# willake/cpu-ray-tracer

Measured on AMD Instinct MI355X. Metric: Mrays/sec (primary+secondary), 1280x720 64spp path trace — pipelined throughput over 878 consecutive 64-spp windows of one progressive render (single_render = one such render alone), higher is better.
Workload: dtype f32; 1 GPU; bunny_scene.xml FileScene BVH-SAH path tracer, 1280x720, 64 spp/step (passes=1, depthLimit=5); 1 step = 64 frames = the next spp window of a progressive render; the 878 steps are one crt_render job (14 render kernel launch(es), a wavefront per (tile, 128 consecutive frames), + ordered accumulate), one sync at the end; triangles=4968, parallelism=tile-wave x1

## Files before the change

cpu-ray-tracer_amd/csrc/device/render_pool.hip:

```cpp
#include <type_traits>
#include "launch.h"
#include "sample_body.h"

namespace crt {

enum : uint32_t {
    F_OX = 0, F_OY, F_OZ, F_DX, F_DY, F_DZ,
    F_RX, F_RY, F_RZ,
    F_T,
    F_SEED, F_META,
    F_U, F_V,
    F_COUNT,
    F_CUR = F_U, F_PEND = F_V,
    F_TRI = F_RX
};
constexpr uint32_t kMetaItemMask = 0x7ffu, kMetaDepthShift = 11u, kMetaInside = 1u << 14, kMetaFresh = 1u << 15, kMetaObjShift = 16u, kMetaLowMask = 0xffffu;
constexpr uint32_t kQueueMask = 127u;

#ifndef CRT_POOL_MIN_WAVES
#define CRT_POOL_MIN_WAVES 4
#endif
#ifndef CRT_POOL_WIDE_MIN_WAVES
#define CRT_POOL_WIDE_MIN_WAVES 4
#endif
#ifndef CRT_POOL_SHADE_MIN
#define CRT_POOL_SHADE_MIN 64
#endif
#ifndef CRT_POOL_NODE_STEPS
#define CRT_POOL_NODE_STEPS 2
#endif
#ifndef CRT_POOL_NODE2_MIN
#define CRT_POOL_NODE2_MIN 16
#endif
#ifndef CRT_POOL_STARVE
#define CRT_POOL_STARVE 40
#endif

#ifdef CRT_POOL_STAMPS
__device__ unsigned long long g_poolStamps[16];
#define CRT_PSTAMP(var) unsigned long long var; asm volatile("s_memtime %0\n\ts_waitcnt lgkmcnt(0)" : "=s"(var) :: "memory")
#define CRT_PACC(i, a, b) (pst[i] += (b) - (a))
#else
#define CRT_PSTAMP(var)
#define CRT_PACC(i, a, b)
#endif
#ifdef CRT_POOL_DENS
__device__ unsigned long long g_poolDens[48];
#define CRT_DENS(i, v) (dens[i] += (uint32_t)(v))
#define CRT_DENS_MASK(i, pred) (dens[i] += (uint32_t)__popcll(__builtin_amdgcn_ballot_w64(pred)))
#define CRT_LIVE_BUCKET(n) ((n) >= 112u ? 0u : (n) >= 96u ? 1u : (n) >= 64u ? 2u : 3u)
#else
#define CRT_DENS(i, v)
#define CRT_DENS_MASK(i, pred)
#endif
#ifdef CRT_POOL_TIMELINE
__device__ unsigned long long* g_poolTimeline = nullptr;
#endif
__device__ __forceinline__ bool lane_in(uint64_t m) { return __builtin_amdgcn_inverse_ballot_w64(m); }
__device__ __forceinline__ uint64_t finite3_mask(f3 v)
{
#ifdef CRT_DIET_NO_MASKS
    const uint32_t m = 0x7f800000u;
    return __builtin_amdgcn_ballot_w64((asu(v.x) & m) != m) & __builtin_amdgcn_ballot_w64((asu(v.y) & m) != m) & __builtin_amdgcn_ballot_w64((asu(v.z) & m) != m);
#else
    const float inf = __builtin_inff();
    return __builtin_amdgcn_fcmpf(__builtin_fabsf(v.x), inf, 4) & __builtin_amdgcn_fcmpf(__builtin_fabsf(v.y), inf, 4) & __builtin_amdgcn_fcmpf(__builtin_fabsf(v.z), inf, 4);
#endif
}
__device__ __forceinline__ uint32_t rank_in(uint64_t m) { return __builtin_amdgcn_mbcnt_hi((uint32_t)(m >> 32), __builtin_amdgcn_mbcnt_lo((uint32_t)m, 0u)); }

template <int KIND, bool COUNT, int S, int REFBITS = 16>
__global__ __launch_bounds__(64, REFBITS == 32 ? CRT_POOL_WIDE_MIN_WAVES : CRT_POOL_MIN_WAVES) void render_pool_kernel(const Scene sc, float4* __restrict__ slab, float* __restrict__ facScratch, Counters* __restrict__ counters,
                                                             unsigned long long* __restrict__ tileClocks, const uint32_t* __restrict__ tileOrder,
                                                             uint32_t tileFirst, uint32_t tileStride, uint32_t tileCount, uint32_t tilesX,
                                                             uint32_t sppFirst, uint32_t frames, uint32_t passes, uint32_t groups, uint32_t waveFrames, const uint32_t* __restrict__ waveTab, uint32_t tabBlocks, uint32_t longFrames,
                                                             uint32_t rankFirst, uint32_t* __restrict__ tileCost, unsigned long long* __restrict__ launchClk, const uint8_t* __restrict__ tileClass)
{
    extern __shared__ uint32_t lds[];
    const uint32_t lane = threadIdx.x;
#ifdef CRT_POOL_TIMELINE
    const unsigned long long tl0 = wall_clock64();
#endif
    const unsigned long long clk0 = (COUNT || tileCost) ? wall_clock64() : 0ull;
    if (launchClk && lane == 0) { atomicMax(&launchClk[0], ~clk0); atomicMax(&launchClk[1], clk0); }
    uint32_t rank0, grp, wf = waveFrames, first = 0u, limit = frames;
    if (waveTab) {
        if (blockIdx.x < tabBlocks) {
            uint32_t lo = 0u, hi = tileCount - rankFirst;
            while (hi - lo > 1u) { const uint32_t mid = (lo + hi) >> 1; if (waveTab[2u * mid] <= blockIdx.x) lo = mid; else hi = mid; }
            rank0 = lo; grp = blockIdx.x - waveTab[2u * lo]; wf = waveTab[2u * lo + 1u]; limit = longFrames;
        } else { const uint32_t b = blockIdx.x - tabBlocks; rank0 = b / groups; grp = b - rank0 * groups; wf = (uint32_t)S; first = longFrames; }
    } else { rank0 = blockIdx.x / groups; grp = blockIdx.x - rank0 * groups; }
    const uint32_t rank = rank0 + rankFirst;
    if (rank >= tileCount) return;
    const uint32_t tl = tileOrder ? tileOrder[rank] : rank;
    const uint32_t frame0 = first + grp * wf;
    if (frame0 >= limit) return;
    const uint32_t nOwn = (limit - frame0 < wf) ? limit - frame0 : wf;
    const uint32_t nStreams = nOwn < (uint32_t)S ? nOwn : (uint32_t)S;
    const uint32_t tile = tileFirst + tl * tileStride;
    const uint32_t tx = tile % tilesX, ty = tile / tilesX;
#ifdef CRT_NO_TILE_CLASS
    constexpr uint32_t tcls = 0u;
#else
    const uint32_t tcls = tileClass ? __builtin_amdgcn_readfirstlane((uint32_t)tileClass[tl]) : 0u;
#endif
    const bool skyTile = tcls == kTileSky;
    const char* __restrict__ geom = sc.geom;
    float* __restrict__ fac = facScratch + (size_t)blockIdx.x * (15u * (uint32_t)S);

    constexpr PoolRefForm R = pool_ref_form((uint32_t)REFBITS);
    using StackEntry = std::conditional_t<REFBITS == 32, uint32_t, uint16_t>;
    constexpr uint32_t kEntryB = (uint32_t)sizeof(StackEntry), kLevelB = 64u * kEntryB;
    char* const ldsB = reinterpret_cast<char*>(lds);
    const uint32_t laneB = lane * kEntryB;
    uint32_t* st = lds + (sc.stackDepth + 1u) * (kLevelB / 4u);
    float* stf = reinterpret_cast<float*>(st);
    uint8_t* qEnd = reinterpret_cast<uint8_t*>(st + F_COUNT * S);
    uint8_t* qBnc = qEnd + 128, * qRdy = qEnd + 256;
    uint16_t* slotFrame = reinterpret_cast<uint16_t*>(qEnd + 384);
    auto stk_top = [&](uint32_t at) -> uint32_t { return *reinterpret_cast<const StackEntry*>(ldsB + at); };
    auto stk_put = [&](uint32_t at, uint32_t v) { *reinterpret_cast<StackEntry*>(ldsB + at) = (StackEntry)v; };

    Cnt cn; cn.rays = cn.primary = cn.interior = cn.leaf = cn.tri = cn.tlas = cn.visits = cn.meshhits = 0;
    uint32_t trips = 0;
#ifdef CRT_POOL_DENS
    uint32_t dens[48]; for (int i = 0; i < 48; i++) dens[i] = 0;
    uint32_t live = nStreams; unsigned long long liveClk = wall_clock64();
#endif
    const uint32_t items = 256u * passes;
    const uint32_t rowLen = 64u * passes;
    const f3 nil3 = mk3(0.0f, 0.0f, 0.0f);

    for (uint32_t s = lane; s < nStreams; s += 64u) {
        st[F_SEED * S + s] = init_seed(tx + ty * (uint32_t)sc.W + (sppFirst + (frame0 + s) * passes) * 1799u);
        st[F_META * S + s] = kMetaFresh;
        qEnd[s] = (uint8_t)s;
        if (S > 64) slotFrame[s] = (uint16_t)s;
    }
    uint32_t nextFrame = nStreams;
    uint32_t endH = 0, endT = nStreams, bncH = 0, bncT = 0, rdyH = 0, rdyT = 0;

    uint64_t mRes = 0ull;
    uint64_t mFinite = ~0ull;
    uint32_t sid = 0, cur = kRefDone, spB = laneB, metaLo = 0u;
    f3 tO = nil3, tD = nil3, trD = nil3;
    Hit h; h.t = 1e34f; h.u = 0; h.v = 0; h.objIdx = -1; h.triIdx = -1;
    rec4 q0 = {0, 0, 0, 0}, q1 = q0, q2 = q0, q3 = q0;

    auto new_ray = [&](auto primary, bool act, uint32_t s, f3 v, bool norm, f3 O, uint32_t seed, uint32_t meta) {
#ifdef CRT_DIET_NO_CAMREL
        constexpr bool PRIM = false;
#else
        constexpr bool PRIM = decltype(primary)::value;
#endif
        constexpr bool FROM_CAM = decltype(primary)::value;
        const bool sky = FROM_CAM && skyTile;
        const bool noLight = FROM_CAM && (tcls & kTileNoLight) != 0u, noFloor = FROM_CAM && (tcls & kTileNoFloor) != 0u, noTree = FROM_CAM && (tcls & kTileNoTree) != 0u;
        f3 D = v, rD = v; Hit nh; nh.t = 1e34f; nh.u = 0; nh.v = 0; nh.objIdx = -1; nh.triIdx = -1;
        uint32_t ncur = kRefDone, pend = 0u;
        if (act) {
            const float inv = rcp_exact(sqrt_exact(dot3(v, v)));
            D = norm ? v * inv : v;
            cn.rays++;
            if (!sky) {
                rD = rcp_exact3(D);
                hit_light_floor<PRIM>(light_floor_from_kernarg<PRIM>(), O, D, nh, noLight, noFloor);
            }
            if (noTree) {
                if (COUNT) { if (KIND == 0) cn.interior++; else cn.tlas++; }
            } else if (sc.rootIsPair) {
                const kernarg_f rp = scene_floats(offsetof(Scene, rootPair));
                const rec4 a0 = {rp[0], rp[1], rp[2], rp[3]}, a1 = {rp[4], rp[5], rp[6], rp[7]};
                const rec4 b0 = {rp[8], rp[9], rp[10], rp[11]}, b1 = {rp[12], rp[13], rp[14], rp[15]};
                float d1, d2;
                const bool allFinite = (__builtin_amdgcn_ballot_w64(true) & ~finite3_mask(rD)) == 0ull;
                if constexpr (PRIM) {
                    const f3 ra0 = mk3(rp[16], rp[17], rp[18]), ra1 = mk3(rp[19], rp[20], rp[21]), rb0 = mk3(rp[22], rp[23], rp[24]), rb1 = mk3(rp[25], rp[26], rp[27]);
                    if (allFinite) { d1 = box_fast_rel(ra0, ra1, rD, nh.t); d2 = box_fast_rel(rb0, rb1, rD, nh.t); }
                    else { d1 = box_exact_rel(ra0, ra1, rD, nh.t); d2 = box_exact_rel(rb0, rb1, rD, nh.t); }
                } else if (allFinite) { d1 = box_fast(a0, a1, O, rD, nh.t); d2 = box_fast(b0, b1, O, rD, nh.t); }
                else { d1 = box_exact(a0, a1, O, rD, nh.t); d2 = box_exact(b0, b1, O, rD, nh.t); }
                const Ordered o = ordered_step(d1, d2, asu(a1.w), asu(b1.w));
                pend = o.push ? o.farRef : 0u;
                ncur = o.hitN ? o.nearRef : kRefDone;
                if (COUNT) { if (KIND == 0) cn.interior++; else cn.tlas++; }
            } else ncur = sc.rootRef16;
            if (COUNT && KIND == 0 && (ncur & R.tagMask) == 0u && ncur != kRefDone) cn.leaf++;
            if (!sky) {
                stf[F_OX * S + s] = O.x; stf[F_OY * S + s] = O.y; stf[F_OZ * S + s] = O.z;
                stf[F_RX * S + s] = rD.x; stf[F_RY * S + s] = rD.y; stf[F_RZ * S + s] = rD.z;
                stf[F_T * S + s] = nh.t;
                st[F_CUR * S + s] = ncur; st[F_PEND * S + s] = pend;
            }
            stf[F_DX * S + s] = D.x; stf[F_DY * S + s] = D.y; stf[F_DZ * S + s] = D.z;
            st[F_SEED * S + s] = seed; st[F_META * S + s] = meta | ((uint32_t)(nh.objIdx + 1) << kMetaObjShift);
        }
        const uint64_t mAct = __builtin_amdgcn_ballot_w64(act);
        uint64_t mW = 0ull, mE = mAct, mB = 0ull;
        if (!sky) {
            const uint32_t depth = (meta >> kMetaDepthShift) & 7u;
            mW = mAct & __builtin_amdgcn_ballot_w64(ncur != kRefDone);
            const uint64_t mStop = __builtin_amdgcn_ballot_w64((uint32_t)(nh.objIdx + 1) <= 1u) | __builtin_amdgcn_ballot_w64((int)depth >= sc.depthLimit);
            mE = mAct & ~mW & mStop; mB = mAct & ~mW & ~mStop;
        }
        CRT_DENS(20, __popcll(mAct)); CRT_DENS(19, __popcll(mW));
        if (!sky) {
            if (lane_in(mW)) qRdy[(rdyT + rank_in(mW)) & kQueueMask] = (uint8_t)s;
            if (lane_in(mB)) qBnc[(bncT + rank_in(mB)) & kQueueMask] = (uint8_t)s;
            rdyT += (uint32_t)__popcll(mW); bncT += (uint32_t)__popcll(mB);
        }
        if (lane_in(mE)) qEnd[(endT + rank_in(mE)) & kQueueMask] = (uint8_t)s;
        endT += (uint32_t)__popcll(mE);
    };
    auto world_ray = [&]() {
        tO = mk3(stf[F_OX * S + sid], stf[F_OY * S + sid], stf[F_OZ * S + sid]);
        tD = mk3(stf[F_DX * S + sid], stf[F_DY * S + sid], stf[F_DZ * S + sid]);
        trD = mk3(stf[F_RX * S + sid], stf[F_RY * S + sid], stf[F_RZ * S + sid]);
    };

    uint64_t mNode2 = 0ull;
    auto node_step = [&](uint64_t m) {
        const bool allFinite = (m & ~mFinite) == 0ull;
        if (lane_in(m)) {
            if (COUNT) { if (KIND == 1 && (cur & R.tlasBit) != 0u) cn.tlas++; else cn.interior++; }
            const uint32_t top = stk_top(spB);
            float d1, d2;
            if (__builtin_expect(allFinite, 1)) { d1 = box_fast(q0, q1, tO, trD, h.t); d2 = box_fast(q2, q3, tO, trD, h.t); }
            else { d1 = box_exact(q0, q1, tO, trD, h.t); d2 = box_exact(q2, q3, tO, trD, h.t); }
            const Ordered o = ordered_step(d1, d2, asu(q1.w), asu(q3.w));
            stk_put(spB + kLevelB, o.farRef);
            const bool pop = !o.hitN && spB != laneB;
            cur = o.hitN ? o.nearRef : (pop ? top : kRefDone);
            spB = spB + (o.push ? kLevelB : 0u) - (pop ? kLevelB : 0u);
            if (COUNT && (cur & R.tagMask) == 0u && cur != kRefDone) cn.leaf++;
        }
    };
    auto record_offset = [&]() -> uint32_t {
        const uint32_t idx = cur & R.indexMask;
        const bool inter = (cur & R.interior) != 0u;
        uint32_t oa = idx * (inter ? 64u : 48u) + (inter ? 0u : sc.leafOff - 48u);
        if (KIND == 1 && (cur & R.tlasBit) != 0u)
            oa = (cur & R.interior) ? sc.instOff + idx * 128u : sc.tlasPairOff + idx * 64u;
        return oa;
    };
    auto load_records = [&](uint64_t m) {
        const uint32_t oa = record_offset();
        if (lane_in(m)) { q0 = ldp<0>(geom, oa); q1 = ldp<1>(geom, oa); q2 = ldp<2>(geom, oa); q3 = ldp<3>(geom, oa); }
    };

    auto tri_step = [&](uint64_t m) {
        CRT_DENS(3, 1); CRT_DENS(4, __popcll(m));
        if (lane_in(m)) {
            if (COUNT) cn.tri++;
            const uint32_t top = stk_top(spB);
            hit_tri(q0, q1, q2, tO, tD, h);
            const bool more = asu(q2.w) > 1u;
            const bool pop = !more && spB != laneB;
            const uint32_t next = more ? cur + 1u : (pop ? top : kRefDone);
            spB -= pop ? kLevelB : 0u;
            if (COUNT && !more && (next & R.tagMask) == 0u && next != kRefDone) cn.leaf++;
            cur = next;
        }
    };

#ifdef CRT_POOL_STAMPS
    unsigned long long pst[12] = {0, 0, 0, 0, 0, 0, 0, 0, 0, 0, 0, 0};
#endif
    for (;;) {
        CRT_PSTAMP(p0);
        if (mRes != 0ull) {
            uint64_t mNode, mTlas = 0ull;
            if (KIND == 0) mNode = mRes & __builtin_amdgcn_ballot_w64(cur > R.interior - 1u);
            else { mTlas = mRes & __builtin_amdgcn_ballot_w64(cur >= R.tlasLeaf); mNode = mRes & __builtin_amdgcn_ballot_w64(cur - R.tlasBit < R.interior); }
            const uint64_t mTri = mRes & ~(mNode | mTlas);
            asm volatile("" : "+v"(q0), "+v"(q1), "+v"(q2), "+v"(q3));
            CRT_DENS(22, __popcll(mRes));
            if (mNode) { CRT_DENS(1, 1); CRT_DENS(2, __popcll(mNode)); }

            if (KIND == 1 && mTlas) { CRT_DENS(23, 1); CRT_DENS(24, __popcll(mTlas)); }
            uint64_t mBack = 0ull;
            if (KIND == 1 && mTlas != 0ull) {
                if (lane_in(mTlas)) {
                    if (COUNT) { cn.tlas++; cn.visits++; }
                    const f3 O = mk3(stf[F_OX * S + sid], stf[F_OY * S + sid], stf[F_OZ * S + sid]);
                    const f3 D = mk3(stf[F_DX * S + sid], stf[F_DY * S + sid], stf[F_DZ * S + sid]);
                    to_object_space(q0, q1, q2, O, D, tO, tD, trD);
                    spB += kLevelB; stk_put(spB, R.ret);
                    const uint32_t next = asu(q3.y);
                    if (COUNT && (next & R.tagMask) == 0u && next != kRefDone) cn.leaf++;
                    cur = next;
                }
                mFinite = (mFinite & ~mTlas) | (mTlas & finite3_mask(trD));
            }
            if (mNode != 0ull) node_step(mNode);
#if CRT_POOL_NODE_STEPS > 1
            uint64_t mLeafNow = 0ull;
#pragma unroll
            for (int rep = 1; rep < CRT_POOL_NODE_STEPS; rep++) {
                const uint64_t mStepped = rep == 1 ? mNode : mNode2;
                mNode2 = mStepped & (KIND == 0 ? __builtin_amdgcn_ballot_w64(cur > R.interior - 1u) : __builtin_amdgcn_ballot_w64(cur - R.tlasBit < R.interior));
                if ((uint32_t)__popcll(mNode2) < (uint32_t)CRT_POOL_NODE2_MIN) { mNode2 = 0ull; break; }
                const uint64_t mLeaf = mStepped & __builtin_amdgcn_ballot_w64((cur & R.tagMask) == 0u) & ~__builtin_amdgcn_ballot_w64(cur == kRefDone);
                load_records(mNode2 | mLeaf);
                mLeafNow |= mLeaf;
                CRT_DENS(28, 1); CRT_DENS(29, __popcll(mNode2));
                node_step(mNode2);
            }
            const uint64_t mTriAll = mTri | mLeafNow;
            const uint64_t mTriRan = mTriAll;
#else
            const uint64_t mTriAll = mTri;
            const uint64_t mTriRan = mTriAll;
#endif
            if (mTriAll != 0ull) tri_step(mTriAll);
            if (KIND == 1) {
                mBack = (mNode | mTriRan) & __builtin_amdgcn_ballot_w64(cur == R.ret);
                if (mBack != 0ull) {
                    if (lane_in(mBack)) {
                        world_ray();
                        const bool pop = spB != laneB;
                        const uint32_t top = stk_top(spB);
                        cur = pop ? top : kRefDone; spB -= pop ? kLevelB : 0u;
                        if (COUNT && (cur & R.tagMask) == 0u && cur != kRefDone) cn.leaf++;
                    }
                    mFinite = (mFinite & ~mBack) | (mBack & finite3_mask(trD));
                }
            }
            asm volatile("" ::: "memory");
            const uint64_t mFin = mRes & __builtin_amdgcn_ballot_w64(cur == kRefDone);
            if (mFin != 0ull) {
                CRT_DENS(5, 1); CRT_DENS(6, __popcll(mFin));
                const uint32_t depth = (metaLo >> kMetaDepthShift) & 7u;
                const uint64_t mStop = __builtin_amdgcn_ballot_w64((uint32_t)(h.objIdx + 1) <= 1u) | __builtin_amdgcn_ballot_w64((int)depth >= sc.depthLimit);
                const uint64_t mE = mFin & mStop, mB = mFin & ~mStop;
                if (lane_in(mFin)) {
                    stf[F_T * S + sid] = h.t; stf[F_U * S + sid] = h.u; stf[F_V * S + sid] = h.v;
                    st[F_TRI * S + sid] = (uint32_t)h.triIdx;
                    st[F_META * S + sid] = metaLo | ((uint32_t)(h.objIdx + 1) << kMetaObjShift);
                }
                if (lane_in(mE)) qEnd[(endT + rank_in(mE)) & kQueueMask] = (uint8_t)sid;
                if (lane_in(mB)) qBnc[(bncT + rank_in(mB)) & kQueueMask] = (uint8_t)sid;
                endT += (uint32_t)__popcll(mE); bncT += (uint32_t)__popcll(mB);
                mRes &= ~mFin;
            }
            asm volatile("" ::: "memory");
        }
        CRT_PSTAMP(p1); CRT_PACC(0, p0, p1);
        if (__builtin_expect(mRes == 0ull, 0)) {
            if ((endT - endH) + (bncT - bncH) + (rdyT - rdyH) == 0u) break;
        }
        if (COUNT) trips++;
        CRT_DENS(0, 1);
#ifdef CRT_POOL_DENS
        dens[32u + CRT_LIVE_BUCKET(live)]++;
#endif
        {
            const uint32_t nRdy = rdyT - rdyH;
            const uint64_t mFree = ~mRes;
            if (nRdy != 0u) if (mFree != 0ull) {
                const uint32_t myRank = rank_in(mFree);
                const uint64_t mTake = mFree & __builtin_amdgcn_ballot_w64(myRank < nRdy);
                CRT_DENS(7, 1); CRT_DENS(8, __popcll(mTake));
                if (lane_in(mTake)) {
                    sid = qRdy[(rdyH + myRank) & kQueueMask];
                    tO = mk3(stf[F_OX * S + sid], stf[F_OY * S + sid], stf[F_OZ * S + sid]);
                    tD = mk3(stf[F_DX * S + sid], stf[F_DY * S + sid], stf[F_DZ * S + sid]);
                    trD = mk3(stf[F_RX * S + sid], stf[F_RY * S + sid], stf[F_RZ * S + sid]);
                    const uint32_t meta = st[F_META * S + sid];
                    h.t = stf[F_T * S + sid]; h.objIdx = (int)(meta >> kMetaObjShift) - 1; h.u = 0; h.v = 0; h.triIdx = -1;
                    metaLo = meta & kMetaLowMask;
                    cur = st[F_CUR * S + sid];
                    const uint32_t pend = st[F_PEND * S + sid];
                    stk_put(laneB + kLevelB, pend);
                    spB = laneB + (pend ? kLevelB : 0u);
                }
                mFinite = (mFinite & ~mTake) | (mTake & finite3_mask(trD));
                mRes |= mTake;
                rdyH += (uint32_t)__popcll(mTake);
            }
            if (mRes != 0ull) {
                CRT_DENS(21, 1);
                uint32_t oa = record_offset();
                if (!lane_in(mRes)) oa = 0u;
                q0 = ldp<0>(geom, oa); q1 = ldp<1>(geom, oa); q2 = ldp<2>(geom, oa); q3 = ldp<3>(geom, oa);
            }
        }
        asm volatile("" ::: "memory");
        {
            const uint32_t nEnd = endT - endH, nBnc = bncT - bncH, nRdy = rdyT - rdyH, nRes = (uint32_t)__popcll(mRes);
            const bool starving = nRes + nRdy < (uint32_t)CRT_POOL_STARVE;
            bool runEnd = false, runBnc = false;
            if ((nEnd | nBnc) >= (uint32_t)CRT_POOL_SHADE_MIN || starving) {
                runEnd = nEnd >= (uint32_t)CRT_POOL_SHADE_MIN || (starving && nEnd > 0u && nEnd >= nBnc);
                runBnc = nBnc >= (uint32_t)CRT_POOL_SHADE_MIN || (starving && nBnc > nEnd);
            }

            CRT_PSTAMP(p2b); CRT_PACC(1, p1, p2b);
            if (runEnd) {
                const uint32_t n = nEnd < 64u ? nEnd : 64u;
                const bool act = lane < n;
                const uint32_t s = act ? qEnd[(endH + lane) & kQueueMask] : 0u;
                endH += n;
                uint32_t meta = 0, seed = 0; int obj = -1; f3 D = nil3;
                if (act) { meta = st[F_META * S + s]; seed = st[F_SEED * S + s]; obj = (int)(meta >> kMetaObjShift) - 1; D = mk3(stf[F_DX * S + s], stf[F_DY * S + s], stf[F_DZ * S + s]); }
                const bool first = (meta & kMetaFresh) != 0u;
                const int depth = (int)((meta >> kMetaDepthShift) & 7u);
                uint32_t item = meta & kMetaItemMask;
                const bool ended = act && !first, miss = ended && obj == -1;
#ifdef CRT_POOL_DENS
                dens[36u + CRT_LIVE_BUCKET(live)]++;
#endif
                CRT_DENS(9, 1); CRT_DENS(10, n); CRT_DENS_MASK(11, miss); CRT_DENS_MASK(13, act && first); CRT_DENS_MASK(25, ended && depth > 0); CRT_DENS_MASK(26, ended && depth > 1); CRT_DENS_MASK(27, ended && depth > 2);
                if (ended && obj >= 2) cn.meshhits++;
                float fk[15];
#pragma unroll
                for (int k = 0; k < 5; k++) {
                    fk[3 * k] = fk[3 * k + 1] = fk[3 * k + 2] = 0.0f;
                    if (!skyTile) if (ended && depth > k) {
#pragma unroll
                        for (int j = 0; j < 3; j++) fk[3 * k + j] = __hip_atomic_load(fac + (3 * k + j) * S + s, __ATOMIC_RELAXED, __HIP_MEMORY_SCOPE_AGENT);
                    }
                }
                uint32_t skyTexel = 0u;
                if (miss) {
                    float phi, theta; sky_angles(D, phi, theta);
                    const kernarg_f sk = scene_floats(offsetof(Scene, skyOffset));
                    skyTexel = sc.texels[tex_index(asu(sk[0]), (int)asu(sk[1]), (int)asu(sk[2]), phi * CRT_INV2PI, theta * CRT_INVPI)];
                }
                bool gen = act && first;
                size_t sampleAt = 0;
                if (ended) {
                    uint32_t pix = item, pass = 0;
                    if (passes != 1u) { pix = item / passes; pass = item - pix * passes; }
                    const uint32_t fr = frame0 + (S > 64 ? (uint32_t)slotFrame[s] : s);
                    sampleAt = (((size_t)(fr >> 6) * tileCount + tl) * 256u + pix) * rowLen + ((fr & 63u) * passes + pass);
                    item++;
                    gen = item < items;
                }
                if (S > 64) if (nextFrame < nOwn) {
                    const uint64_t mDone = __builtin_amdgcn_ballot_w64(ended) & ~__builtin_amdgcn_ballot_w64(gen);
                    if (mDone != 0ull) {
                        const uint32_t f = nextFrame + rank_in(mDone);
                        const uint64_t mTake = mDone & __builtin_amdgcn_ballot_w64(f < nOwn);
                        if (lane_in(mTake)) {
                            slotFrame[s] = (uint16_t)f;
                            seed = init_seed(tx + ty * (uint32_t)sc.W + (sppFirst + (frame0 + f) * passes) * 1799u);
                            item = 0u; gen = true;
                        }
                        nextFrame += (uint32_t)__popcll(mTake);
                    }
                }
#ifdef CRT_POOL_DENS
                {
                    const uint32_t gone = (uint32_t)__popcll(__builtin_amdgcn_ballot_w64(ended) & ~__builtin_amdgcn_ballot_w64(gen));
                    if (gone) { const unsigned long long now = wall_clock64(); dens[44u + CRT_LIVE_BUCKET(live)] += (uint32_t)(now - liveClk); liveClk = now; live -= gone; }
                }
#endif
                const kernarg_f cam = scene_floats(offsetof(Scene, camPos));
                const f3 camPos = mk3(cam[0], cam[1], cam[2]);
                f3 v = camPos;
                if (gen) {
                    const uint32_t pix = (passes == 1u) ? item : item / passes;
                    const f3 TL = mk3(cam[3], cam[4], cam[5]);
#ifdef CRT_DIET_NO_CAMREL
                    const f3 TR = mk3(cam[6], cam[7], cam[8]), BL = mk3(cam[9], cam[10], cam[11]);
                    const f3 right = TR - TL, down = BL - TL;
#else
                    constexpr size_t pc = (offsetof(Scene, primRight) - offsetof(Scene, camPos)) / 4;
                    const f3 right = mk3(cam[pc], cam[pc + 1], cam[pc + 2]), down = mk3(cam[pc + 3], cam[pc + 4], cam[pc + 5]);
#endif
                    v = primary_target(camPos, TL, right, down, cam[12], cam[13], tx, ty, pix, seed);
                    cn.primary++;
                }
                CRT_DENS_MASK(12, gen);
                CRT_PSTAMP(e1); CRT_PACC(2, p2b, e1);
                new_ray(std::true_type{}, gen, s, v, true, camPos, seed, item);
                CRT_PSTAMP(e2); CRT_PACC(3, e1, e2);
                if (ended) {
                    f3 L = miss ? tex_unpack(skyTexel) : ((depth >= sc.depthLimit) ? mk3(0, 0, 0) : mk3(24, 24, 22));
                    if (!skyTile) {
#pragma unroll
                        for (int k = 4; k >= 0; k--)
                            if (depth > k) L = mk3(fk[3 * k], fk[3 * k + 1], fk[3 * k + 2]) * L;
                    }
                    slab[sampleAt] = make_float4(L.x, L.y, L.z, 0.0f);
                }
#ifdef CRT_POOL_STAMPS
                { CRT_PSTAMP(e3); CRT_PACC(4, e2, e3); pst[10]++; }
#endif
                asm volatile("" :: "v"(fk[0]), "v"(fk[1]), "v"(fk[2]), "v"(fk[3]), "v"(fk[4]), "v"(fk[5]), "v"(fk[6]), "v"(fk[7]), "v"(fk[8]), "v"(fk[9]), "v"(fk[10]), "v"(fk[11]), "v"(fk[12]), "v"(fk[13]), "v"(fk[14]), "v"(skyTexel));
            }
            CRT_PSTAMP(p3);
            asm volatile("" ::: "memory");
            if (runBnc) {
                const uint32_t n = nBnc < 64u ? nBnc : 64u;
                const bool act = lane < n;
                const uint32_t s = act ? qBnc[(bncH + lane) & kQueueMask] : 0u;
                bncH += n;
                f3 O = nil3, D = nil3; float ht = 0, hu = 0, hv = 0; int obj = 1; uint32_t tri = 0, seed = 0, meta = 0;
                if (act) {
                    tri = st[F_TRI * S + s];
                    O = mk3(stf[F_OX * S + s], stf[F_OY * S + s], stf[F_OZ * S + s]);
                    D = mk3(stf[F_DX * S + s], stf[F_DY * S + s], stf[F_DZ * S + s]);
                    ht = stf[F_T * S + s]; hu = stf[F_U * S + s]; hv = stf[F_V * S + s];
                    seed = st[F_SEED * S + s]; meta = st[F_META * S + s]; obj = (int)(meta >> kMetaObjShift) - 1;
                }
                const bool mesh = act && obj >= 2;
#ifdef CRT_POOL_DENS
                dens[40u + CRT_LIVE_BUCKET(live)]++;
#endif
                CRT_DENS(14, 1); CRT_DENS(15, n); CRT_DENS_MASK(16, mesh);
                rec4 s0 = {0, 0, 0, 0}, s1 = s0, s2 = s0, s3 = s0;
                if (mesh) { const uint32_t so = sc.shadeOff + tri * 64u; s0 = ldp<0>(geom, so); s1 = ldp<1>(geom, so); s2 = ldp<2>(geom, so); s3 = ldp<3>(geom, so); cn.meshhits++; }
                const bool inside = (meta & kMetaInside) != 0u;
                const int depth = (int)((meta >> kMetaDepthShift) & 7u);
                const uint32_t item = meta & kMetaItemMask;
                f3 v = O; bool newInside = false;
                if (act) {
                    const f3 I = O + ht * D;
                    SurfPoint p;
                    if (obj == 1) {
                        const kernarg_f fl = scene_floats(offsetof(Scene, floorN));
                        const kernarg_f fm = scene_floats(offsetof(Scene, floorMat));
                        const rec4 m0 = {fm[0], fm[1], fm[2], fm[3]}, m1 = {fm[4], fm[5], fm[6], fm[7]};
                        p = floor_point(mk3(fl[0], fl[1], fl[2]), fl[4], m0, m1, I);
                    } else p = mesh_point<KIND>(s0, s1, s2, s3, hu, hv, obj, geom, sc.instOff, sc.mats);
                    const f3 N = face_ray(p.N, D);
                    uint32_t texel = 0x00ffffffu;
                    if (p.tW > 0) texel = sc.texels[tex_index(p.tOff, p.tW, p.tH, p.tu, p.tv)];
                    const f3 medium = medium_of(inside, p.absorb, ht);
                    CRT_PSTAMP(b1); CRT_PACC(5, p3, b1);
                    const Bounce b = draw_bounce(seed, D, N, inside, p.refl, p.refr);
                    newInside = b.newInside;
                    const f3 c = (p.tW > 0) ? tex_unpack(texel) : mk3(1.0f, 1.0f, 1.0f);
                    CRT_PSTAMP(b2); CRT_PACC(6, b1, b2);
                    const float inv = rcp_exact(sqrt_exact(dot3(b.v, b.v)));
                    const f3 nv = b.branch == kDiffuse ? b.v * inv : b.v;
                    v = nv;
                    const f3 factor = bounce_factor(b.branch, c, medium, nv, N);
                    float* fd = fac + (3 * depth) * S + s;
                    __hip_atomic_store(fd, factor.x, __ATOMIC_RELAXED, __HIP_MEMORY_SCOPE_AGENT);
                    __hip_atomic_store(fd + S, factor.y, __ATOMIC_RELAXED, __HIP_MEMORY_SCOPE_AGENT);
                    __hip_atomic_store(fd + 2 * S, factor.z, __ATOMIC_RELAXED, __HIP_MEMORY_SCOPE_AGENT);
                    O = I + nv * CRT_EPS;
                    CRT_PSTAMP(b3); CRT_PACC(7, b2, b3);
                }
                CRT_PSTAMP(b4);
                new_ray(std::false_type{}, act, s, v, false, O, seed, item | ((uint32_t)(depth + 1) << kMetaDepthShift) | (newInside ? kMetaInside : 0u));
#ifdef CRT_POOL_STAMPS
                { CRT_PSTAMP(b5); CRT_PACC(8, b4, b5); pst[11]++; }
#endif
                asm volatile("" :: "v"(s0), "v"(s1), "v"(s2), "v"(s3));
            }
#ifdef CRT_POOL_STAMPS
            pst[9]++;
#endif
        }
    }
#ifdef CRT_POOL_STAMPS
    if (lane == 0) for (int i = 0; i < 12; i++) atomicAdd(&g_poolStamps[i], pst[i]);
#endif
#ifdef CRT_POOL_DENS
    dens[44u + CRT_LIVE_BUCKET(live)] += (uint32_t)(wall_clock64() - liveClk);
    if (lane == 0) for (int i = 0; i < 48; i++) if (dens[i]) atomicAdd(&g_poolDens[i], (unsigned long long)dens[i]);
#endif

#ifdef CRT_POOL_TIMELINE
    if (lane == 0 && g_poolTimeline) { uint32_t hw; asm volatile("s_getreg_b32 %0, hwreg(HW_REG_HW_ID)" : "=s"(hw)); g_poolTimeline[3 * (size_t)blockIdx.x] = tl0; g_poolTimeline[3 * (size_t)blockIdx.x + 1] = wall_clock64(); g_poolTimeline[3 * (size_t)blockIdx.x + 2] = hw; }
#endif
    if (tileCost && lane == 0 && nOwn == (uint32_t)S) atomicMax(&tileCost[tl], (uint32_t)((wall_clock64() - clk0) * 64ull / (uint32_t)S));
    if (launchClk && lane == 0) { const unsigned long long now = wall_clock64(), last = __hip_atomic_load(&launchClk[1], __ATOMIC_RELAXED, __HIP_MEMORY_SCOPE_AGENT), from = last > clk0 ? last : clk0; if (now > from) atomicAdd(&launchClk[2], now - from); }
    if (COUNT && tileClocks && lane == 0 && nOwn == frames) {
        tileClocks[2 * tl] = wall_clock64() - clk0;
        tileClocks[2 * tl + 1] = trips;
    }
    uint32_t vals[8] = {cn.rays, cn.primary, cn.interior, cn.leaf, cn.tri, cn.tlas, cn.visits, cn.meshhits};
#pragma unroll
    for (int i = 0; i < 8; i++) {
        if (!COUNT && i >= 2 && i != 7) continue;
        uint32_t sum = wave_sum(vals[i]);
        if (lane == 0 && sum) atomicAdd(&counters->v[i], (unsigned long long)sum);
    }
}

}

#ifndef CRT_POOL_STREAMS
#define CRT_POOL_STREAMS 128
#endif
extern "C" uint32_t crt_pool_streams(uint32_t frames) { return frames > 64u ? (uint32_t)CRT_POOL_STREAMS : 64u; }
#ifndef CRT_POOL_EXTRA_LDS
#define CRT_POOL_EXTRA_LDS 0
#endif
extern "C" uint32_t crt_pool_lds_bytes(uint32_t stackDepth, uint32_t streams, uint32_t refBits) { return (stackDepth + 1u) * 64u * (refBits / 8u) + crt::F_COUNT * streams * 4u + 3u * 128u + (streams > 64u ? 2u * streams : 0u) + (uint32_t)CRT_POOL_EXTRA_LDS; }
extern "C" uint32_t crt_pool_lds_limit(int device)
{
    static uint32_t known[64] = {};
    if (device >= 0 && device < 64 && known[device]) return known[device];
    int v = 0;
    if (hipDeviceGetAttribute(&v, hipDeviceAttributeMaxSharedMemoryPerBlock, device) != hipSuccess || v <= 0) { (void)hipGetLastError(); return 0u; }
    const uint32_t limit = (uint32_t)v < 64u * 1024u ? (uint32_t)v : 64u * 1024u;
    if (device >= 0 && device < 64) known[device] = limit;
    return limit;
}
extern "C" size_t crt_pool_scratch_bytes_per_window(uint32_t tileCount) { return (size_t)tileCount * 128u * 15u * 4u; }

#ifdef CRT_POOL_STAMPS
extern "C" int crt_debug_pool_stamps(unsigned long long* out, int reset)
{
    if (out && hipMemcpyFromSymbol(out, HIP_SYMBOL(crt::g_poolStamps), 128) != hipSuccess) return -1;
    if (reset) { unsigned long long z[16] = {}; if (hipMemcpyToSymbol(HIP_SYMBOL(crt::g_poolStamps), z, 128) != hipSuccess) return -1; }
    return 0;
}
#endif
#ifdef CRT_POOL_DENS
extern "C" int crt_debug_pool_density(unsigned long long* out, int reset)
{
    if (out && hipMemcpyFromSymbol(out, HIP_SYMBOL(crt::g_poolDens), 384) != hipSuccess) return -1;
    if (reset) { unsigned long long z[48] = {}; if (hipMemcpyToSymbol(HIP_SYMBOL(crt::g_poolDens), z, 384) != hipSuccess) return -1; }
    return 0;
}
#endif
#ifdef CRT_POOL_TIMELINE
static unsigned long long* g_timelineHost = nullptr; static size_t g_timelineCount = 0;
extern "C" size_t crt_debug_pool_timeline(unsigned long long* out, size_t cap)
{
    const size_t n = g_timelineCount < cap ? g_timelineCount : cap;
    if (out && n) (void)hipMemcpy(out, g_timelineHost, n * 24, hipMemcpyDeviceToHost);
    return g_timelineCount;
}
#endif
extern "C" hipError_t crt_launch_render_pool(const crt::Scene* sc, void* slab, void* facScratch, crt::Counters* counters, unsigned long long* tileClocks, const uint32_t* tileOrder,
                                             uint32_t tileFirst, uint32_t tileStride, uint32_t tileCount, uint32_t tilesX, uint32_t sppFirst,
                                             uint32_t frames, uint32_t passes, int collectStats, uint32_t rankFirst, uint32_t waveFrames, const uint32_t* waveTab, uint32_t tabBlocks, uint32_t longFrames,
                                             uint32_t* tileCost, unsigned long long* launchClk, const uint8_t* tileClass, uint32_t extraLds, hipStream_t stream)
{
    if (tileCount == 0 || frames == 0) return hipSuccess;
    if (sc->poolRefBits != 16u && sc->poolRefBits != 32u) return hipErrorInvalidValue;
    const uint32_t S = crt_pool_streams(frames);
    const uint32_t wf = (S == 64u || waveFrames < S) ? S : waveFrames;
    if (wf % S != 0u || wf > 0xff80u) return hipErrorInvalidValue;
    if (S == 64u) waveTab = nullptr;
    if (waveTab && (tabBlocks == 0u || longFrames == 0u || longFrames > frames)) return hipErrorInvalidValue;
    const uint32_t groups = waveTab ? (frames - longFrames + S - 1u) / S : (frames + wf - 1u) / wf;
    if ((unsigned long long)tileCount * ((frames + S - 1u) / S) > 0x7fffffffull) return hipErrorInvalidValue;
    if (rankFirst >= tileCount) return hipSuccess;
    dim3 grid(waveTab ? tabBlocks + (tileCount - rankFirst) * groups : (tileCount - rankFirst) * groups), block(64);
#ifdef CRT_POOL_TIMELINE
    { static unsigned long long* buf = nullptr; static size_t cap = 0;
      if (cap < (size_t)grid.x) { if (buf) (void)hipFree(buf); (void)hipMalloc((void**)&buf, (size_t)grid.x * 24); cap = grid.x; (void)hipMemcpyToSymbol(HIP_SYMBOL(crt::g_poolTimeline), &buf, sizeof(buf)); }
      (void)hipMemsetAsync(buf, 0, (size_t)grid.x * 24, stream); g_timelineHost = buf; g_timelineCount = grid.x; }
#endif
    const uint32_t ldsBytes = crt_pool_lds_bytes(sc->stackDepth, S, sc->poolRefBits) + extraLds;
    { int dev = 0; if (hipGetDevice(&dev) != hipSuccess) return hipGetLastError(); if (ldsBytes > crt_pool_lds_limit(dev)) return hipErrorInvalidValue; }
#define CRT_LAUNCH(K, C, SS) do { if (sc->poolRefBits == 32u) CRT_LAUNCH_R(K, C, SS, 32); else CRT_LAUNCH_R(K, C, SS, 16); } while (0)
#define CRT_LAUNCH_R(K, C, SS, RB) hipLaunchKernelGGL((crt::render_pool_kernel<K, C, SS, RB>), grid, block, ldsBytes, stream, *sc, (float4*)slab, (float*)facScratch, counters, tileClocks, tileOrder, tileFirst, tileStride, tileCount, tilesX, sppFirst, frames, passes, groups, wf, waveTab, tabBlocks, longFrames, rankFirst, tileCost, launchClk, tileClass)
#define CRT_LAUNCH_S(K, C) do { if (S == 64u) CRT_LAUNCH(K, C, 64); else CRT_LAUNCH(K, C, CRT_POOL_STREAMS); } while (0)
    if (sc->kind == 0) { if (collectStats) CRT_LAUNCH_S(0, true); else CRT_LAUNCH_S(0, false); }
    else { if (collectStats) CRT_LAUNCH_S(1, true); else CRT_LAUNCH_S(1, false); }
#undef CRT_LAUNCH_S
#undef CRT_LAUNCH
#undef CRT_LAUNCH_R
    return hipGetLastError();
}
```

Before: 31340 Mrays/s.

## Keep wavefront pool control decisions scalar and specialize node steps on finiteness

Reworks the persistent pool kernel's control flow so lane masks come straight from scalar compares (uicmp/sicmp) rather than ballots over per-lane bools. Sky checks, pass counts and the shading-pass decision are pinned into SGPRs. The node traversal is split into two compiled variants, one assuming all inverse directions are finite (the common case) and one exact fallback. A live-stream counter replaces the queue-empty exit check, and the end-pass refill logic is restructured around masks. The aim is to cut VALU and ballot overhead and divergent branching in the scheduler loop, at the cost of code duplication and some subtle correctness risk in the rewritten termination logic.

```diff
diff --git a/cpu-ray-tracer_amd/csrc/device/render_pool.hip b/cpu-ray-tracer_amd/csrc/device/render_pool.hip
--- a/cpu-ray-tracer_amd/csrc/device/render_pool.hip
+++ b/cpu-ray-tracer_amd/csrc/device/render_pool.hip
@@ -67,6 +67,19 @@
     return __builtin_amdgcn_fcmpf(__builtin_fabsf(v.x), inf, 4) & __builtin_amdgcn_fcmpf(__builtin_fabsf(v.y), inf, 4) & __builtin_amdgcn_fcmpf(__builtin_fabsf(v.z), inf, 4);
 #endif
 }
+#define CRT_CTL_SEQ() asm volatile("")
+__device__ __forceinline__ bool ctl_free(uint64_t mRes) { CRT_CTL_SEQ(); return mRes != ~0ull; }
+#ifdef CRT_CTL_NO_DECIDE
+__device__ __forceinline__ uint32_t fresh(uint32_t x) { return x; }
+#else
+__device__ __forceinline__ uint32_t fresh(uint32_t x) { asm("" : "+s"(x)); return x; }
+#endif
+__device__ __forceinline__ uint32_t pop32(uint64_t m) { uint32_t n = (uint32_t)__builtin_popcountll(m); asm("" : "+s"(n)); return n; }
+__device__ __forceinline__ uint64_t mask_ne(uint32_t a, uint32_t b) { return __builtin_amdgcn_uicmp(a, b, 33); }
+__device__ __forceinline__ uint64_t mask_eq(uint32_t a, uint32_t b) { return __builtin_amdgcn_uicmp(a, b, 32); }
+__device__ __forceinline__ uint64_t mask_ult(uint32_t a, uint32_t b) { return __builtin_amdgcn_uicmp(a, b, 36); }
+__device__ __forceinline__ uint64_t mask_ule(uint32_t a, uint32_t b) { return __builtin_amdgcn_uicmp(a, b, 37); }
+__device__ __forceinline__ uint64_t mask_sge(int a, int b) { return __builtin_amdgcn_sicmp(a, b, 39); }
 __device__ __forceinline__ uint32_t rank_in(uint64_t m) { return __builtin_amdgcn_mbcnt_hi((uint32_t)(m >> 32), __builtin_amdgcn_mbcnt_lo((uint32_t)m, 0u)); }
 
 template <int KIND, bool COUNT, int S, int REFBITS = 16>
@@ -105,7 +118,12 @@
 #else
     const uint32_t tcls = tileClass ? __builtin_amdgcn_readfirstlane((uint32_t)tileClass[tl]) : 0u;
 #endif
+#if defined(CRT_CTL_NO_DECIDE) || defined(CRT_NO_TILE_CLASS)
     const bool skyTile = tcls == kTileSky;
+    auto not_sky = [&]() -> bool { return !skyTile; };
+#else
+    auto not_sky = [&]() -> bool { return fresh(tcls) != kTileSky; };
+#endif
     const char* __restrict__ geom = sc.geom;
     float* __restrict__ fac = facScratch + (size_t)blockIdx.x * (15u * (uint32_t)S);
 
@@ -138,6 +156,9 @@
         qEnd[s] = (uint8_t)s;
         if (S > 64) slotFrame[s] = (uint16_t)s;
     }
+#ifndef CRT_CTL_NO_DECIDE
+    uint32_t nLive = nStreams;
+#endif
     uint32_t nextFrame = nStreams;
     uint32_t endH = 0, endT = nStreams, bncH = 0, bncT = 0, rdyH = 0, rdyT = 0;
 
@@ -148,14 +169,13 @@
     Hit h; h.t = 1e34f; h.u = 0; h.v = 0; h.objIdx = -1; h.triIdx = -1;
     rec4 q0 = {0, 0, 0, 0}, q1 = q0, q2 = q0, q3 = q0;
 
-    auto new_ray = [&](auto primary, bool act, uint32_t s, f3 v, bool norm, f3 O, uint32_t seed, uint32_t meta) {
+    auto new_ray = [&](auto primary, uint64_t mActIn, bool act, uint32_t s, f3 v, bool norm, f3 O, uint32_t seed, uint32_t meta) {
 #ifdef CRT_DIET_NO_CAMREL
         constexpr bool PRIM = false;
 #else
         constexpr bool PRIM = decltype(primary)::value;
 #endif
         constexpr bool FROM_CAM = decltype(primary)::value;
-        const bool sky = FROM_CAM && skyTile;
         const bool noLight = FROM_CAM && (tcls & kTileNoLight) != 0u, noFloor = FROM_CAM && (tcls & kTileNoFloor) != 0u, noTree = FROM_CAM && (tcls & kTileNoTree) != 0u;
         f3 D = v, rD = v; Hit nh; nh.t = 1e34f; nh.u = 0; nh.v = 0; nh.objIdx = -1; nh.triIdx = -1;
         uint32_t ncur = kRefDone, pend = 0u;
@@ -163,7 +183,7 @@
             const float inv = rcp_exact(sqrt_exact(dot3(v, v)));
             D = norm ? v * inv : v;
             cn.rays++;
-            if (!sky) {
+            if (!FROM_CAM || not_sky()) {
                 rD = rcp_exact3(D);
                 hit_light_floor<PRIM>(light_floor_from_kernarg<PRIM>(), O, D, nh, noLight, noFloor);
             }
@@ -187,7 +207,7 @@
                 if (COUNT) { if (KIND == 0) cn.interior++; else cn.tlas++; }
             } else ncur = sc.rootRef16;
             if (COUNT && KIND == 0 && (ncur & R.tagMask) == 0u && ncur != kRefDone) cn.leaf++;
-            if (!sky) {
+            if (!FROM_CAM || not_sky()) {
                 stf[F_OX * S + s] = O.x; stf[F_OY * S + s] = O.y; stf[F_OZ * S + s] = O.z;
                 stf[F_RX * S + s] = rD.x; stf[F_RY * S + s] = rD.y; stf[F_RZ * S + s] = rD.z;
                 stf[F_T * S + s] = nh.t;
@@ -196,20 +216,27 @@
             stf[F_DX * S + s] = D.x; stf[F_DY * S + s] = D.y; stf[F_DZ * S + s] = D.z;
             st[F_SEED * S + s] = seed; st[F_META * S + s] = meta | ((uint32_t)(nh.objIdx + 1) << kMetaObjShift);
         }
+#ifdef CRT_CTL_NO_BALLOT
         const uint64_t mAct = __builtin_amdgcn_ballot_w64(act);
+#else
+        const uint64_t mAct = mActIn;
+#endif
         uint64_t mW = 0ull, mE = mAct, mB = 0ull;
-        if (!sky) {
+        if (!FROM_CAM || not_sky()) {
             const uint32_t depth = (meta >> kMetaDepthShift) & 7u;
+#ifdef CRT_CTL_NO_BALLOT
             mW = mAct & __builtin_amdgcn_ballot_w64(ncur != kRefDone);
             const uint64_t mStop = __builtin_amdgcn_ballot_w64((uint32_t)(nh.objIdx + 1) <= 1u) | __builtin_amdgcn_ballot_w64((int)depth >= sc.depthLimit);
+#else
+            mW = mAct & mask_ne(ncur, kRefDone);
+            const uint64_t mStop = mask_ule((uint32_t)(nh.objIdx + 1), 1u) | mask_sge((int)depth, sc.depthLimit);
+#endif
             mE = mAct & ~mW & mStop; mB = mAct & ~mW & ~mStop;
-        }
-        CRT_DENS(20, __popcll(mAct)); CRT_DENS(19, __popcll(mW));
-        if (!sky) {
             if (lane_in(mW)) qRdy[(rdyT + rank_in(mW)) & kQueueMask] = (uint8_t)s;
             if (lane_in(mB)) qBnc[(bncT + rank_in(mB)) & kQueueMask] = (uint8_t)s;
             rdyT += (uint32_t)__popcll(mW); bncT += (uint32_t)__popcll(mB);
         }
+        CRT_DENS(20, __popcll(mAct)); CRT_DENS(19, __popcll(mW));
         if (lane_in(mE)) qEnd[(endT + rank_in(mE)) & kQueueMask] = (uint8_t)s;
         endT += (uint32_t)__popcll(mE);
     };
@@ -220,8 +247,12 @@
     };
 
     uint64_t mNode2 = 0ull;
-    auto node_step = [&](uint64_t m) {
+    auto node_step = [&](auto exactTag, uint64_t m) {
+#ifdef CRT_CTL_NO_FINITE
         const bool allFinite = (m & ~mFinite) == 0ull;
+#else
+        constexpr bool allFinite = !decltype(exactTag)::value;
+#endif
         if (lane_in(m)) {
             if (COUNT) { if (KIND == 1 && (cur & R.tlasBit) != 0u) cn.tlas++; else cn.interior++; }
             const uint32_t top = stk_top(spB);
@@ -293,26 +324,39 @@
                 }
                 mFinite = (mFinite & ~mTlas) | (mTlas & finite3_mask(trD));
             }
-            if (mNode != 0ull) node_step(mNode);
+            uint64_t mLeafNow = 0ull;
+            auto node_phase = [&](auto exactTag) {
+                if (mNode != 0ull) node_step(exactTag, mNode);
 #if CRT_POOL_NODE_STEPS > 1
-            uint64_t mLeafNow = 0ull;
 #pragma unroll
-            for (int rep = 1; rep < CRT_POOL_NODE_STEPS; rep++) {
-                const uint64_t mStepped = rep == 1 ? mNode : mNode2;
-                mNode2 = mStepped & (KIND == 0 ? __builtin_amdgcn_ballot_w64(cur > R.interior - 1u) : __builtin_amdgcn_ballot_w64(cur - R.tlasBit < R.interior));
-                if ((uint32_t)__popcll(mNode2) < (uint32_t)CRT_POOL_NODE2_MIN) { mNode2 = 0ull; break; }
-                const uint64_t mLeaf = mStepped & __builtin_amdgcn_ballot_w64((cur & R.tagMask) == 0u) & ~__builtin_amdgcn_ballot_w64(cur == kRefDone);
-                load_records(mNode2 | mLeaf);
-                mLeafNow |= mLeaf;
-                CRT_DENS(28, 1); CRT_DENS(29, __popcll(mNode2));
-                node_step(mNode2);
-            }
+                for (int rep = 1; rep < CRT_POOL_NODE_STEPS; rep++) {
+                    const uint64_t mStepped = rep == 1 ? mNode : mNode2;
+                    mNode2 = mStepped & (KIND == 0 ? __builtin_amdgcn_ballot_w64(cur > R.interior - 1u) : __builtin_amdgcn_ballot_w64(cur - R.tlasBit < R.interior));
+#ifdef CRT_CTL_NO_DECIDE
+                    if ((uint32_t)__popcll(mNode2) < (uint32_t)CRT_POOL_NODE2_MIN) { mNode2 = 0ull; break; }
+#else
+                    if (pop32(mNode2) < (uint32_t)CRT_POOL_NODE2_MIN) { mNode2 = 0ull; break; }
+#endif
+                    const uint64_t mLeaf = mStepped & __builtin_amdgcn_ballot_w64((cur & R.tagMask) == 0u) & ~__builtin_amdgcn_ballot_w64(cur == kRefDone);
+                    load_records(mNode2 | mLeaf);
+                    mLeafNow |= mLeaf;
+                    CRT_DENS(28, 1); CRT_DENS(29, __popcll(mNode2));
+                    node_step(exactTag, mNode2);
+                }
+#endif
+            };
+#ifdef CRT_CTL_NO_FINITE
+            node_phase(std::false_type{});
+#else
+            if (mNode != 0ull) {
+                uint64_t mInf = mNode & ~mFinite, mInf2 = mInf;
+                asm("" : "+s"(mInf2));
+                if (__builtin_expect(mInf == 0ull, 1)) node_phase(std::false_type{});
+                if (__builtin_expect(mInf2 != 0ull, 0)) node_phase(std::true_type{});
+            }
+#endif
             const uint64_t mTriAll = mTri | mLeafNow;
             const uint64_t mTriRan = mTriAll;
-#else
-            const uint64_t mTriAll = mTri;
-            const uint64_t mTriRan = mTriAll;
-#endif
             if (mTriAll != 0ull) tri_step(mTriAll);
             if (KIND == 1) {
                 mBack = (mNode | mTriRan) & __builtin_amdgcn_ballot_w64(cur == R.ret);
@@ -347,18 +391,27 @@
             asm volatile("" ::: "memory");
         }
         CRT_PSTAMP(p1); CRT_PACC(0, p0, p1);
+#ifdef CRT_CTL_NO_DECIDE
         if (__builtin_expect(mRes == 0ull, 0)) {
             if ((endT - endH) + (bncT - bncH) + (rdyT - rdyH) == 0u) break;
         }
+#endif
         if (COUNT) trips++;
         CRT_DENS(0, 1);
+#ifdef CRT_POOL_STAMPS
+        pst[9]++;
+#endif
 #ifdef CRT_POOL_DENS
         dens[32u + CRT_LIVE_BUCKET(live)]++;
 #endif
         {
             const uint32_t nRdy = rdyT - rdyH;
             const uint64_t mFree = ~mRes;
+#ifdef CRT_CTL_NO_DECIDE
             if (nRdy != 0u) if (mFree != 0ull) {
+#else
+            if (nRdy != 0u) if (ctl_free(mRes)) {
+#endif
                 const uint32_t myRank = rank_in(mFree);
                 const uint64_t mTake = mFree & __builtin_amdgcn_ballot_w64(myRank < nRdy);
                 CRT_DENS(7, 1); CRT_DENS(8, __popcll(mTake));
@@ -387,27 +440,49 @@
             }
         }
         asm volatile("" ::: "memory");
+        const uint32_t nEnd = endT - endH, nBnc = bncT - bncH;
+#ifdef CRT_CTL_NO_DECIDE
         {
-            const uint32_t nEnd = endT - endH, nBnc = bncT - bncH, nRdy = rdyT - rdyH, nRes = (uint32_t)__popcll(mRes);
+            const uint32_t nRdy = rdyT - rdyH, nRes = (uint32_t)__popcll(mRes);
             const bool starving = nRes + nRdy < (uint32_t)CRT_POOL_STARVE;
             bool runEnd = false, runBnc = false;
             if ((nEnd | nBnc) >= (uint32_t)CRT_POOL_SHADE_MIN || starving) {
                 runEnd = nEnd >= (uint32_t)CRT_POOL_SHADE_MIN || (starving && nEnd > 0u && nEnd >= nBnc);
                 runBnc = nBnc >= (uint32_t)CRT_POOL_SHADE_MIN || (starving && nBnc > nEnd);
             }
+#else
+        static_assert(CRT_POOL_SHADE_MIN == 64, "the pass decision's shifts assume a threshold of 64");
+        uint32_t walking = pop32(mRes) + (rdyT - rdyH), fullest = nEnd | nBnc;
+        asm("" : "+s"(walking));
+        walking = fullest >= 64u ? 0u : walking;
+        asm("" : "+s"(walking), "+s"(fullest));
+        if (walking < (uint32_t)CRT_POOL_STARVE) {
+            const uint32_t run = fullest >= 64u ? (nEnd >> 6) | ((nBnc >> 6) << 8) : (nEnd >= nBnc ? nEnd : nBnc << 8);
+            const uint32_t runEnd = run & 0xffu, runBnc = run >> 8;
+#endif
 
             CRT_PSTAMP(p2b); CRT_PACC(1, p1, p2b);
-            if (runEnd) {
+            if (runEnd != 0u) {
                 const uint32_t n = nEnd < 64u ? nEnd : 64u;
+#ifdef CRT_CTL_NO_BALLOT
                 const bool act = lane < n;
+#else
+                const uint64_t mActE = mask_ult(lane, n);
+                const bool act = lane_in(mActE);
+#endif
                 const uint32_t s = act ? qEnd[(endH + lane) & kQueueMask] : 0u;
                 endH += n;
                 uint32_t meta = 0, seed = 0; int obj = -1; f3 D = nil3;
                 if (act) { meta = st[F_META * S + s]; seed = st[F_SEED * S + s]; obj = (int)(meta >> kMetaObjShift) - 1; D = mk3(stf[F_DX * S + s], stf[F_DY * S + s], stf[F_DZ * S + s]); }
-                const bool first = (meta & kMetaFresh) != 0u;
                 const int depth = (int)((meta >> kMetaDepthShift) & 7u);
                 uint32_t item = meta & kMetaItemMask;
+#ifdef CRT_CTL_NO_BALLOT
+                const bool first = (meta & kMetaFresh) != 0u;
                 const bool ended = act && !first, miss = ended && obj == -1;
+#else
+                const uint64_t mFirst = mask_ne(meta & kMetaFresh, 0u), mEnded = mActE & ~mFirst, mMiss = mEnded & mask_eq(meta >> kMetaObjShift, 0u);
+                const bool first = lane_in(mFirst), ended = lane_in(mEnded), miss = lane_in(mMiss);
+#endif
 #ifdef CRT_POOL_DENS
                 dens[36u + CRT_LIVE_BUCKET(live)]++;
 #endif
@@ -417,7 +492,7 @@
 #pragma unroll
                 for (int k = 0; k < 5; k++) {
                     fk[3 * k] = fk[3 * k + 1] = fk[3 * k + 2] = 0.0f;
-                    if (!skyTile) if (ended && depth > k) {
+                    if (not_sky()) if (ended && depth > k) {
 #pragma unroll
                         for (int j = 0; j < 3; j++) fk[3 * k + j] = __hip_atomic_load(fac + (3 * k + j) * S + s, __ATOMIC_RELAXED, __HIP_MEMORY_SCOPE_AGENT);
                     }
@@ -432,12 +507,13 @@
                 size_t sampleAt = 0;
                 if (ended) {
                     uint32_t pix = item, pass = 0;
-                    if (passes != 1u) { pix = item / passes; pass = item - pix * passes; }
+                    if (fresh(passes) != 1u) { pix = item / passes; pass = item - pix * passes; }
                     const uint32_t fr = frame0 + (S > 64 ? (uint32_t)slotFrame[s] : s);
                     sampleAt = (((size_t)(fr >> 6) * tileCount + tl) * 256u + pix) * rowLen + ((fr & 63u) * passes + pass);
                     item++;
                     gen = item < items;
                 }
+#ifdef CRT_CTL_NO_BALLOT
                 if (S > 64) if (nextFrame < nOwn) {
                     const uint64_t mDone = __builtin_amdgcn_ballot_w64(ended) & ~__builtin_amdgcn_ballot_w64(gen);
                     if (mDone != 0ull) {
@@ -451,6 +527,32 @@
                         nextFrame += (uint32_t)__popcll(mTake);
                     }
                 }
+                const uint64_t mGen = __builtin_amdgcn_ballot_w64(gen);
+#ifndef CRT_CTL_NO_DECIDE
+                { const uint64_t mGone = __builtin_amdgcn_ballot_w64(ended) & ~mGen; if (mGone != 0ull) nLive -= pop32(mGone); }
+#endif
+#else
+                uint64_t mGen = mFirst | (mEnded & mask_ult(item, items));
+                const uint64_t mDone = mEnded & ~mGen;
+                if (mDone != 0ull) {
+                    uint64_t mTake = 0ull;
+                    if (S > 64) if (nextFrame < nOwn) {
+                        const uint32_t f = nextFrame + rank_in(mDone);
+                        mTake = mDone & mask_ult(f, nOwn);
+                        if (lane_in(mTake)) {
+                            slotFrame[s] = (uint16_t)f;
+                            seed = init_seed(tx + ty * (uint32_t)sc.W + (sppFirst + (frame0 + f) * passes) * 1799u);
+                            item = 0u;
+                        }
+                        nextFrame += pop32(mTake);
+                        mGen |= mTake;
+                    }
+#ifndef CRT_CTL_NO_DECIDE
+                    nLive -= pop32(mDone & ~mTake);
+#endif
+                }
+                gen = lane_in(mGen);
+#endif
 #ifdef CRT_POOL_DENS
                 {
                     const uint32_t gone = (uint32_t)__popcll(__builtin_amdgcn_ballot_w64(ended) & ~__builtin_amdgcn_ballot_w64(gen));
@@ -461,7 +563,7 @@
                 const f3 camPos = mk3(cam[0], cam[1], cam[2]);
                 f3 v = camPos;
                 if (gen) {
-                    const uint32_t pix = (passes == 1u) ? item : item / passes;
+                    const uint32_t pix = (fresh(passes) == 1u) ? item : item / passes;
                     const f3 TL = mk3(cam[3], cam[4], cam[5]);
 #ifdef CRT_DIET_NO_CAMREL
                     const f3 TR = mk3(cam[6], cam[7], cam[8]), BL = mk3(cam[9], cam[10], cam[11]);
@@ -475,11 +577,11 @@
                 }
                 CRT_DENS_MASK(12, gen);
                 CRT_PSTAMP(e1); CRT_PACC(2, p2b, e1);
-                new_ray(std::true_type{}, gen, s, v, true, camPos, seed, item);
+                new_ray(std::true_type{}, mGen, gen, s, v, true, camPos, seed, item);
                 CRT_PSTAMP(e2); CRT_PACC(3, e1, e2);
                 if (ended) {
                     f3 L = miss ? tex_unpack(skyTexel) : ((depth >= sc.depthLimit) ? mk3(0, 0, 0) : mk3(24, 24, 22));
-                    if (!skyTile) {
+                    if (not_sky()) {
 #pragma unroll
                         for (int k = 4; k >= 0; k--)
                             if (depth > k) L = mk3(fk[3 * k], fk[3 * k + 1], fk[3 * k + 2]) * L;
@@ -493,9 +595,15 @@
             }
             CRT_PSTAMP(p3);
             asm volatile("" ::: "memory");
-            if (runBnc) {
+            if (runBnc != 0u) {
                 const uint32_t n = nBnc < 64u ? nBnc : 64u;
+#ifdef CRT_CTL_NO_BALLOT
                 const bool act = lane < n;
+                const uint64_t mActB = 0ull;
+#else
+                const uint64_t mActB = mask_ult(lane, n);
+                const bool act = lane_in(mActB);
+#endif
                 const uint32_t s = act ? qBnc[(bncH + lane) & kQueueMask] : 0u;
                 bncH += n;
                 f3 O = nil3, D = nil3; float ht = 0, hu = 0, hv = 0; int obj = 1; uint32_t tri = 0, seed = 0, meta = 0;
@@ -547,16 +655,16 @@
                     CRT_PSTAMP(b3); CRT_PACC(7, b2, b3);
                 }
                 CRT_PSTAMP(b4);
-                new_ray(std::false_type{}, act, s, v, false, O, seed, item | ((uint32_t)(depth + 1) << kMetaDepthShift) | (newInside ? kMetaInside : 0u));
+                new_ray(std::false_type{}, mActB, act, s, v, false, O, seed, item | ((uint32_t)(depth + 1) << kMetaDepthShift) | (newInside ? kMetaInside : 0u));
 #ifdef CRT_POOL_STAMPS
                 { CRT_PSTAMP(b5); CRT_PACC(8, b4, b5); pst[11]++; }
 #endif
                 asm volatile("" :: "v"(s0), "v"(s1), "v"(s2), "v"(s3));
             }
-#ifdef CRT_POOL_STAMPS
-            pst[9]++;
-#endif
         }
+#ifndef CRT_CTL_NO_DECIDE
+        if (nLive == 0u) break;
+#endif
     }
 #ifdef CRT_POOL_STAMPS
     if (lane == 0) for (int i = 0; i < 12; i++) atomicAdd(&g_poolStamps[i], pst[i]);
```

New measurement: 32270 Mrays/s, median of 6. 3.0% higher.
